# qwerty35/swarm_simulator

Hardware: AMD Instinct MI355X
Metric: agent-trajectories/sec (RBP plan: SFC+RSFC+QP) (higher is better)
Workload: dtype f64

## Files before the change

### swarm_simulator_amd/csrc/kernels/knot_lds.inc

```
#pragma once
#include "knot_panel_layout.h"

#define KL_LD 38
#define KL_LDU 50
#define KL_I 40
#ifndef KL_XCH
#define KL_XCH 6
#endif
typedef __attribute__((address_space(3))) double kl_lds;
typedef __attribute__((address_space(3))) int kl_ldsi;
typedef double kl_d2 __attribute__((ext_vector_type(2)));
typedef __attribute__((address_space(3))) kl_d2 kl_lds2;
typedef double kl_d4 __attribute__((ext_vector_type(4)));

__host__ __device__ constexpr int kl_area_doubles(int nk) {
    return ((nk + 1) * KL_LDU + (nk + 1) * KL_LD + KL_I + 1) & ~1;
}

template <int NK>
struct KlArea {
    static constexpr int NT = (NK + 15) / 16;
    static constexpr int C = 0, CSZ = (NK + 1) * KL_LDU;
    static constexpr int MX = CSZ, MXSZ = (NK + 1) * KL_LD;
    static constexpr int I = MX + MXSZ;
// ... 562 lines not shown
        return dinv;
    } else {
#pragma unroll
        for (int k = 0; k < NK; ++k) m[k] = (k == r) ? 1.0 : 0.0;
        if (FOLLOW)
            kl_follow_LinvT<NK>(m, C, I, P, pbase);
        else
            kl_row_times_LinvT<NK>(m, C, I);
        if (FOLLOW) kl_await_opaque(P, pbase + NK + 1);
        const double dinv = I[act ? r : 0];
        kl_store_rows<NK>(m, MX, r, act);
        if (FOLLOW) kl_publish(Mdone, done_value);
        return dinv;
    }
}
```

### swarm_simulator_amd/csrc/kernels/qp.hip

```cpp
#include <algorithm>
#include <type_traits>
#include <vector>

#include "rbp_dev.h"

#pragma clang fp contract(fast)

#include "knot_lds.inc"
#include "common/ipm_rows.h"

#ifndef QP_THREADS
#define QP_THREADS 512
#endif
#define QP_MAX_ITERS 80
#ifndef QP_WARM_TAU
#define QP_WARM_TAU 1e-3
#endif
#ifndef QP_MU0
#define QP_MU0 3e-1
#endif
#ifndef QP_ROW_UNROLL
#define QP_ROW_UNROLL 2
#endif
#ifndef QP_ROW_PF
// ... 25 lines not shown
#endif
#ifndef QP_WAVES_PER_EU
#define QP_WAVES_PER_EU 2
#endif
#ifndef QP_CHAIN_PRIO
#define QP_CHAIN_PRIO 3
#endif
#ifndef QP_STAGE_BUFS
#define QP_STAGE_BUFS (QP_THREADS >= 512 ? 3 : 2)
#endif
#ifndef QP_STAGE_REGS
#define QP_STAGE_REGS (QP_THREADS >= 512 ? 0 : 2)
#endif
#ifndef QP_MID_FOLLOW
#define QP_MID_FOLLOW (QP_THREADS >= 512)
#endif
#ifndef QP_EARLY_TRIES
#define QP_EARLY_TRIES 2
#endif
#ifndef QP_EARLY_TOL
#define QP_EARLY_TOL 1e-6
#endif
#include "lh_layout.h"
#define PL_NC 256
#define PL_PMAX 160
#define PL_PBIG 192
__host__ __device__ inline int polish_pmax(int nk) { return nk <= 36 ? 112 : PL_PMAX; }
__host__ __device__ inline size_t polish_s_doubles(int nj) { return std::max((size_t)PL_NC * PL_NC, ipm::k0g_doubles(nj)); }
__host__ __device__ inline size_t polish_ws_doubles(int nj, int nk) {
    return 18 * (size_t)nj + 2 + ipm::k0g_doubles(nj) + PL_NC * 14 + polish_s_doubles(nj) + 8 + lhp_size(PL_PBIG) + 4 * 6 * PL_PBIG + 3 * (size_t)nj * nk;
// ... 1392 lines not shown
    c.w = carve(ws_base + (size_t)mission * ws_stride, c.d, nbmax);
    double* ctrl = S.ctrl + (size_t)mission * N * 3 * 6 * MS;
    c.ctrl = ctrl;
    c.normals = S.rsfc_normal + (size_t)mission * S.npair * MS * 3;
    c.radius = S.radius + (size_t)mission * N;
    const QpDims& d = c.d;
    const QpWs& w = c.w;
    const double* T = S.T + (size_t)mission * (MS + 1);
    double* scal = S.scalars + (size_t)mission * SC_N;

    extern __shared__ __attribute__((aligned(16))) double lds_raw[];
    double* red = lds_raw;
    int* flag = (int*)(lds_raw + 16);
    double* lds = lds_raw + 32;
#ifdef QP_PROFILE
    const BlkArgs ba{d.nk, d.nj, d.ldb, c.lds_avail, w.Td, w.To, w.Lf, w.Ek, scal};
#else
    const BlkArgs ba{d.nk, d.nj, d.ldb, c.lds_avail, w.Td, w.To, w.Lf, w.Ek, nullptr};
#endif

    PROF_DECL;
    int frozen_free_rows = 0, nfar = 0;
    if (!qp_setup_batch(S, c, ctrl, T, mission, first, nb, flag, lds, frozen_free_rows, far_R, nfar)) return 0;
    PROF(8);
    PassIO io;
    __shared__ RowCtx c_lds;
#if QP_ROW_BLK > 0
    __shared__ SweepMeta meta_lds;
    const bool meta_ok = nb * d.M <= QP_META_G && d.ntile + 1 <= 16 && d.N <= 256 && (size_t)nb * d.M * d.N < 65536;
    __syncthreads();
    if (meta_ok) {
        for (int rk = tid; rk < nb * d.M; rk += QP_THREADS) {
            const int g = w.fperm[rk];
// ... 13 lines not shown
    const double pin_viol = block_reduce(io.vmax, 1, red);
    if (pin_viol > 1e-6) {
        if (tid == 0) {
            atomicCAS(&S.status[mission], 0, (int)RBP_ERR_QP_FAILED);
#ifndef QP_PROFILE
            scal[SC_PROF0 + 1] = 1000.0 * batch + 1, scal[SC_PROF0 + 2] = pin_viol;
#endif
        }
        return 0;
    }
    const double nrows_free = (double)((size_t)(d.oq - 6) * (6 * d.nb + d.npb)) + (double)frozen_free_rows;
    bool ok = false;
    int it_count = 0, polished = 0, early_tries = 0, fail_reason = 3;
    double gap_next = 0, pres_next = 0, kkt_ipm = 0;
    double flops = 0, rows_swept = 0, row_bytes = 0, sweep_bytes = 0;
    const double blk_doubles = d.nk <= 36 ? 5.0 * (d.nk * (d.nk + 1) / 2) + 5.0 * d.nk : 8.0 * d.ldb * d.ldb;
    const double bytes_sweeps = 88.0 * frozen_free_rows + 64.0 * (double)(d.oq - 6) * (6.0 * d.nb + 2.0 * d.npb) + 288.0 * (double)d.nb * (d.oq - 6);
    const double bytes_iter = bytes_sweeps + 8.0 * (double)d.nj * blk_doubles;
    const PolishWs pw = polish_carve(w.polish, d.nj);
    row_pass<PASS_INIT>(c, io);
    __threadfence_block();
    __syncthreads();
#ifdef QP_TRACE
    double* trc = S.coef + (size_t)mission * N * 3 * 6 * MS;
#endif
    for (int iter = 0; iter < QP_MAX_ITERS; ++iter) {
        it_count = iter;
        PROF(0);
        if (iter == 0) {
            io.sum0 = 0, io.vmax = 0;
            SWEEP(PASS_BUILD);
// ... 31 lines not shown
            const int acc = polish_entry(c, pw, lds, red, flag, polish_first ? 1 : 0);
            __syncthreads();
            PROF(0);
#ifdef QP_POLSTATS
            if (tid == 0 && !polish_first) scal[25] += (early_tries == 1), scal[26] += (early_tries == 1 && acc == 0), scal[27] += (early_tries == 2), scal[29] += (early_tries == 2 && acc == 0);
#endif
            if (acc == 0) {
                ok = true, polished = 1;
                break;
            }
        }
        if (d.nk > 36)
            assemble_blocks(c, lds);
        else if (ASM_HELPERS == 0 && !QP_FOLLOW_ASM)
            assemble_blocks_lds(asm_args(c), d.nj, lds);
        PROF(3);
        __threadfence_block();
        __syncthreads();
        TRC(5, trc_sum(w.Td, (size_t)d.nj * d.ldb * d.ldb, red));
        if (!factor_entry(ba, asm_args(c), lds, flag)) {
            fail_reason = 2;
            break;
        }
        flops += d.nk <= 36 ? (double)d.nj * ((7.0 / 6.0) * d.nk * (double)d.nk * d.nk + 6.0 * d.nk * (double)d.nk)
                            : (double)d.nj * (7.0 / 3.0) * d.nk * (double)d.nk * d.nk;
        PROF(4);
        TRC(6, trc_sum(d.nk <= 36 ? w.Lf : w.Td, d.nk <= 36 ? (size_t)d.nj * 2 * d.nk * d.nk : (size_t)d.nj * d.ldb * d.ldb, red));
#ifndef QP_TRACE
        if (d.nk <= 36) {
            PROF(5);
            solve_entry(ba, w.rhs, lds, SolveOut{w.dxa, w.Lk, d.oq, 1, w.cpacc, w.rbase, 0.0});
            PROF(6);
        } else
#endif
        {
            rhs_from_acc(c, false, 0.0);
            __threadfence_block();
            __syncthreads();
            PROF(5);
            TRC(7, trc_sum(w.rhs, (size_t)d.nj * d.nk, red));
            solve_entry(ba, w.rhs, lds);
            PROF(6);
            TRC(8, trc_sum(w.rhs, (size_t)d.nj * d.nk, red));
            apply_F(d, w, w.rhs, w.dxa);
            __threadfence_block();
            __syncthreads();
// ... 303 lines not shown
```

### swarm_simulator_amd/csrc/kernels/qp_base.inc

```

#ifdef QP_PROFILE
#define PROF_DECL long long prof_t0 = wall_clock64(), prof_acc[12] = {0, 0, 0, 0, 0, 0, 0, 0, 0, 0, 0, 0}
#define PROF(i)                                \
    do {                                       \
        __syncthreads();                       \
        long long t_ = wall_clock64();         \
        prof_acc[i] += t_ - prof_t0;           \
        prof_t0 = t_;                          \
    } while (0)
#define PROF_FLUSH(scal)                                                         \
    do {                                                                         \
        if (threadIdx.x == 0)                                                    \
            for (int i_ = 0; i_ < 12; ++i_) scal[SC_PROF0 + i_] += (double)prof_acc[i_]; \
    } while (0)
#else
#define PROF_DECL
#define PROF(i)
#define PROF_FLUSH(scal)
#endif

struct QpDims {
    int N, M, oq;
    int nb, NF, npb;
    int nk, nj, ld;
// ... 117 lines not shown
    v = wave_red(v, op);
    const int wave = threadIdx.x >> 6, lane = threadIdx.x & 63;
    if (lane == 0) red[wave] = v;
    __syncthreads();
    double r = red[0];
    for (int i = 1; i < QP_THREADS / 64; ++i) r = red_op(r, red[i], op);
    __syncthreads();
    return r;
}

struct BlkArgs {
    int nk, nj, ldb, lds_avail;
    double *Td, *To, *Lf;
    double* Ek;
    double* prof;
};
__device__ __forceinline__ int uni(int v) { return __builtin_amdgcn_readfirstlane(v); }
template <class T>
__device__ __forceinline__ T* uni(T* p) {
    const unsigned long long v = (unsigned long long)p;
    const unsigned lo = __builtin_amdgcn_readfirstlane((unsigned)v), hi = __builtin_amdgcn_readfirstlane((unsigned)(v >> 32));
    return (T*)(((unsigned long long)hi << 32) | lo);
}
__device__ __forceinline__ void blk_unpack(const BlkArgs& b, QpDims& d, QpWs& w) {
    d = QpDims{};
    w = QpWs{};
    d.nk = uni(b.nk), d.nj = uni(b.nj), d.ldb = uni(b.ldb), d.ld = d.nk + 1;
    w.Td = uni(b.Td), w.To = uni(b.To), w.Lf = uni(b.Lf), w.Ek = uni(b.Ek), w.prof = uni(b.prof);
}
template <class T>
__device__ __forceinline__ T uni_words(const T& v) {
    static_assert(sizeof(T) % 4 == 0, "whole words");
    union U {
        T t;
        unsigned wd[sizeof(T) / 4];
        __device__ U() {}
    } in, out;
    in.t = v;
#pragma unroll
    for (unsigned i = 0; i < sizeof(T) / 4; ++i) out.wd[i] = __builtin_amdgcn_readfirstlane(in.wd[i]);
    return out.t;
}

// ... 48 lines not shown
```

### swarm_simulator_amd/csrc/kernels/qp_wave_factor.inc

```

__device__ __forceinline__ int twist_mid(int nj) { return nj / 2; }

#define ASM_WAVE0 4
#define ASM_HELPERS (QP_THREADS / 64 > ASM_WAVE0 ? QP_THREADS / 64 - ASM_WAVE0 : 0)
#ifndef QP_FOLLOW_ASM
#define QP_FOLLOW_ASM (ASM_HELPERS == 0)
#endif
#define ASMF_READY(cnt, h) ((kl_ldsi*)((cnt) + 76 + (h)))
__device__ __forceinline__ void wait_blocks(int* cnt, int i) {
    while (__hip_atomic_load(cnt + i, __ATOMIC_RELAXED, __HIP_MEMORY_SCOPE_WORKGROUP) < ASM_HELPERS) __builtin_amdgcn_s_sleep(2);
    __builtin_amdgcn_fence(__ATOMIC_ACQUIRE, "workgroup");
}

typedef double d4 __attribute__((ext_vector_type(4)));

template <int NK>
__device__ __forceinline__ bool chol_rows(double (&a)[NK], double& dinv) {
    bool ok = true;
    const int r = threadIdx.x & 63;
    dinv = 1.0;
#pragma unroll
    for (int c = 0; c < NK; ++c) {
        const double dcc = rl(a[c], c);
        if (!(dcc > 0)) ok = false;
// ... 96 lines not shown

#if defined(QP_PROFILE) && !defined(QP_LHSTATS) && !defined(QP_SOLVE_TIMERS)
#define CHAIN_TW(cnt, slot) ((__attribute__((address_space(3))) unsigned long long*)((cnt) + 96) + ((slot) - 25))
#define CHAIN_T0 long long ct_ = wall_clock64()
#define CHAIN_T(slot)                                                                                                                              \
    do {                                                                                                                                           \
        const long long t_ = wall_clock64();                                                                                                       \
        __hip_atomic_fetch_add(CHAIN_TW(cnt, slot), (dir > 0 && r == 0) ? (unsigned long long)(t_ - ct_) : 0ull, __ATOMIC_RELAXED, __HIP_MEMORY_SCOPE_WORKGROUP); \
        ct_ = t_;                                                                                                                                  \
    } while (0)
#define CHAIN_FLUSH()                                                                                   \
    do {                                                                                                \
        kl_sync();                                                                                      \
        if (w.prof && dir > 0 && r == 0)                                                                \
            for (int k_ = 25; k_ < 28; ++k_) w.prof[k_] += (double)(long long)*CHAIN_TW(cnt, k_);       \
    } while (0)
#else
#define CHAIN_T0
#define CHAIN_T(slot)
#define CHAIN_FLUSH()
#endif
#define CHAIN_SYNC(cnt, h) ((kl_ldsi*)((cnt) + 64 + 2 * (h)))
#define ASM_CONSUMED(cnt, h) ((kl_ldsi*)((cnt) + 72 + (h)))

template <int NK>
__device__ __forceinline__ bool wave_factor_chain(const QpDims& d, const QpWs& w, int j0, int count, int dir, double* ldsW, int* cnt, int h) {
    using A = KlArea<NK>;
    kl_lds* base = (kl_lds*)ldsW;
    kl_lds *MX = base + A::MX, *I = base + A::I, *U = base + A::C;
    kl_ldsi *P = CHAIN_SYNC(cnt, h), *Mdone = P + 1;
    const int r = threadIdx.x & 63;
    const bool act = r < NK;
    const int rr = act ? r : 0;
    bool ok = true;
    int seen = 0, seen_img = 0;
    if constexpr (kl_fused_path(NK)) {
        double cf[KlPanels<NK>::NT][3];
        for (int i = 0, j = j0; i < count; ++i, j += dir) {
            CHAIN_T0;
            kl_d4 s[KlPanels<NK>::TILES];
            kl_tiles_zero<NK>(s);
            if (i > 0) {
                kl_await(Mdone, i, seen);
                CHAIN_T(27);
                kl_fused_update<NK>(s, MX, I, r, cf);
            }
            CHAIN_T(25);
            if (QP_FOLLOW_ASM)
                kl_await(ASMF_READY(cnt, h), i + 1, seen_img);
            else
                wait_blocks(cnt, i);
            CHAIN_T(26);
            fused_coupling_coef<NK>(w, j, dir, r, cf);
            const kl_lds* Timg = ASM_HELPERS > 0 ? (const kl_lds*)(ldsW - (size_t)h * A::SIZE + 2 * A::SIZE + 128 + (size_t)(h + 2 * (i & 1)) * ASML_DOUBLES(NK, (NK / 9)))
                                 : QP_FOLLOW_ASM ? (const kl_lds*)(ldsW - (size_t)h * A::SIZE + 2 * A::SIZE + 128 + (size_t)h * ASML_DOUBLES(NK, (NK / 9)))
                                                 : nullptr;
            if (!knot_ldl_add<NK>(w, j, s, base, r, P, i * (NK + 1), Timg, ASM_CONSUMED(cnt, h), i + 1)) ok = false;
            CHAIN_T(27);
        }
        CHAIN_FLUSH();
        return ok;
    }
    for (int i = 0, j = j0; i < count; ++i, j += dir) {
        CHAIN_T0;
        if (i > 0) kl_syrk<NK>(MX, I, U, r, false);
        CHAIN_T(25);
        if (QP_FOLLOW_ASM)
            kl_await(ASMF_READY(cnt, h), i + 1, seen_img);
        else
            wait_blocks(cnt, i);
        CHAIN_T(26);
        double e0, e1, e2, x[NK];
        coupling_coef(w, j, dir, rr, e0, e1, e2);
// ... 44 lines not shown
        kl_await(ASMF_READY(cnt, 0), mid + 1, seen_img);
    } else {
        wait_blocks(cnt, cnt_idx);
    }
    kl_ldsi* scratch = CHAIN_SYNC(cnt, 2);
    const kl_lds* Timg = ASM_HELPERS > 0 ? (const kl_lds*)(ldsL + 2 * A::SIZE + 128 + (size_t)(2 * (cnt_idx & 1)) * ASML_DOUBLES(NK, (NK / 9)))
                         : QP_FOLLOW_ASM ? (const kl_lds*)(ldsL + 2 * A::SIZE + 128) : nullptr;
    bool ok;
    if constexpr (kl_fused_path(NK))
        ok = knot_ldl_add<NK>(w, mid, s, bl, r, scratch, 0, Timg);
    else
        ok = knot_ldl<NK>(w, mid, nsy > 0, bl, r, act, rr, scratch, 0, Timg);
    if (!QP_MID_FOLLOW) {
        int seen = 0;
        knot_inverse<NK, false>(w, mid, bl, r, act, scratch, 0, seen, scratch, 0);
    }
    return ok;
}

template <int NK, int ROLE>
__device__ __forceinline__ bool twisted_factor(const QpDims& d, const QpWs& w, int* flag, double* lds, const AsmArgs* asmb) {
    const int wave = (ROLE == 0 || ROLE == 2) ? (threadIdx.x >> 6) & 1 : 4, mid = twist_mid(d.nj);
    const int nl = mid, nr = d.nj - 1 - mid, SF = nl > nr ? nl : nr;
    constexpr int AREA = KlArea<NK>::SIZE;
    int* cnt = (int*)(lds + 2 * AREA);
    static_assert((QP_MAX_M - 1) / 2 + 1 <= 64, "cnt[0..SF] must end below CHAIN_SYNC (cnt + 64): sessions with M > QP_MAX_M are refused");
    if (threadIdx.x == 0) *flag = 0;
    __syncthreads();
    bool ok = true;
    for (int i = threadIdx.x; i < 2 * AREA + 64; i += QP_THREADS) lds[i] = 0.0;
// ... 85 lines not shown
```

### swarm_simulator_amd/csrc/kernels/qp_wave_solve.inc

```

#define KS_VPAD 16
#define KS_VLEN (KS_VPAD + KL_I + KS_VPAD)
template <int NK>
struct KsPieces {
    static constexpr int CH = (NK * 15 + 35) / 36;
    static constexpr int N0 = NK, N1 = NK - CH > 0 ? NK - CH : 0, N2 = NK - 2 * CH > 0 ? NK - 2 * CH : 0;
    static_assert(NK - 3 * CH <= 0 && N0 + N1 + N2 <= 64, "three chunks, one wavefront");
    static_assert(3 * CH - NK <= KS_VPAD && 3 * CH - 1 - (NK - 1) <= KS_VPAD, "vector padding");
    __device__ static __forceinline__ void of_lane(int lane, int& idx, int& t) {
        t = lane < N0 ? 0 : (lane < N0 + N1 ? 1 : 2);
        idx = lane < N0 ? lane : (lane < N0 + N1 ? lane - N0 : (lane < N0 + N1 + N2 ? lane - N0 - N1 : 0));
    }
};
template <int NK>
__device__ __forceinline__ double kl_matvec_cols(const kl_lds* Mst, const kl_lds* b, kl_lds* psum, int lane) {
    using P = KsPieces<NK>;
    int idx, t;
    P::of_lane(lane, idx, t);
    const int k0 = P::CH * t, c = k0 + idx;
    const kl_lds* mp = Mst + k0 * KL_LD + c;
    const kl_lds* bp = b + k0;
    double mv[P::CH], bv[P::CH];
#pragma unroll
    for (int j = 0; j < P::CH; ++j) mv[j] = mp[j * KL_LD], bv[j] = bp[j];
    double s0 = 0, s1 = 0, s2 = 0;
#pragma unroll
    for (int j = 0; j < P::CH; ++j) {
        if (j % 3 == 0) s0 += mv[j] * bv[j];
        if (j % 3 == 1) s1 += mv[j] * bv[j];
        if (j % 3 == 2) s2 += mv[j] * bv[j];
    }
    psum[lane] = (s0 + s1) + s2;
    kl_sync();
    const int cc = lane < NK ? lane : 0;
    double r = psum[cc];
    if (P::N1 > 0) r += cc >= P::CH ? psum[P::N0 + cc - P::CH] : 0.0;
    if (P::N2 > 0) r += cc >= 2 * P::CH ? psum[P::N0 + P::N1 + cc - 2 * P::CH] : 0.0;
    return r;
}
template <int NK>
__device__ __forceinline__ double kl_matvec_rows(const kl_lds* Mst, const kl_lds* b, kl_lds* psum, int lane) {
    using P = KsPieces<NK>;
    int idx, t;
    P::of_lane(lane, idx, t);
    const int k0 = NK - P::CH * (t + 1);
    const kl_lds* mp = Mst + idx * KL_LD + k0;
    const kl_lds* bp = b + k0;
    double mv[P::CH], bv[P::CH];
#pragma unroll
    for (int j = 0; j < P::CH; ++j) mv[j] = mp[j], bv[j] = bp[j];
    double s0 = 0, s1 = 0, s2 = 0;
#pragma unroll
    for (int j = 0; j < P::CH; ++j) {
        if (j % 3 == 0) s0 += mv[j] * bv[j];
        if (j % 3 == 1) s1 += mv[j] * bv[j];
        if (j % 3 == 2) s2 += mv[j] * bv[j];
    }
    psum[lane] = (s0 + s1) + s2;
    kl_sync();
    const int rr = lane < NK ? lane : 0;
    double r = psum[rr];
    if (P::N1 > 0) r += rr < P::N1 ? psum[P::N0 + rr] : 0.0;
    if (P::N2 > 0) r += rr < P::N2 ? psum[P::N0 + P::N1 + rr] : 0.0;
    return r;
}

template <int NK>
struct KsLayout {
    static constexpr int SM = NK * KL_LD, SCH = SM + KL_I, STG = 2 * SCH;
    static constexpr int LEAD = 16;
    static constexpr int VECS = 6 * KS_VLEN + 2 * 64;
};

struct SolveOut {
    double* dx_out;
    const double* Lk;
    int oq;
    int rhs_mode = 0;
    const double* cpacc = nullptr;
    const double* rbase = nullptr;
    double sigma_mu = 0;
};
template <int NK, int ROLE>
__device__ __forceinline__ void solve_staged(const QpDims& d, const QpWs& w, double* rhs, double* lds, SolveOut so = SolveOut{nullptr, nullptr, 0}) {
    using KS = KsLayout<NK>;
    constexpr int STG = KS::STG, SCH = KS::SCH, SM = KS::SM;
    const int tid = threadIdx.x, nj = d.nj, mid = twist_mid(nj);
    const int nl = mid, nr = nj - 1 - mid, SF = nl > nr ? nl : nr;
    const int nsteps = 2 * SF + 1;
    lds += KS::LEAD;
    kl_lds* vec = (kl_lds*)(lds + QP_STAGE_BUFS * STG);
    kl_lds* small = vec + ((nj * NK + 1) & ~1);
    if (so.rhs_mode) {
        constexpr int nu = NK / 3;
        const int oq = so.oq;
        const size_t ncp = (size_t)(NK / 9) * oq;
        const bool corrector = so.rhs_mode == 2;
        for (int it = tid; it < nj * nu; it += QP_THREADS) {
            const int j = it / nu + 1, u = it % nu, a = u / 3, k = u % 3;
            double g[6];
#pragma unroll
            for (int q = 0; q < 6; ++q) {
                const int j6 = 6 * (j - 1) + 3 + q;
                const __attribute__((address_space(1))) double* ac = QGC(so.cpacc) + (size_t)a * oq + j6;
                g[q] = corrector ? ac[k * ncp] - so.sigma_mu * ac[(3 + k) * ncp] : ac[(6 + k) * ncp];
            }
            const __attribute__((address_space(1))) double* L = QGC(so.Lk) + 9 * j;
            const size_t o0 = (size_t)(j - 1) * NK + u * 3;
// ... 25 lines not shown
                const int side = e >= NE, idx = side ? e - NE : e;
                if (idx < NTRI) {
                    int rw = (int)(((2 * NK + 1) - sqrtf((float)((2 * NK + 1) * (2 * NK + 1) - 8 * idx))) * 0.5f);
                    if (rw * NK - rw * (rw - 1) / 2 > idx) rw--;
                    if ((rw + 1) * NK - (rw + 1) * rw / 2 <= idx) rw++;
                    const int k = rw + idx - (rw * NK - rw * (rw - 1) / 2);
                    soff[u] = rw * NK + k, doff[u] = side * SCH + rw * KL_LD + k;
                } else {
                    soff[u] = NK * NK + (idx - NTRI), doff[u] = side * SCH + SM + (idx - NTRI);
                }
            }
        }
    }
    for (int i = tid; i < KS::LEAD + QP_STAGE_BUFS * STG; i += QP_THREADS) (lds - KS::LEAD)[i] = 0.0;
    __syncthreads();
    auto stage = [&](int s, double* buf) {
        const int jl = left_j(s), jr = right_j(s);
        const double* srcl = w.Lf + (size_t)(jl >= 0 ? jl : 0) * KF_STRIDE(NK);
        const double* srcr = w.Lf + (size_t)(jr >= 0 ? jr : 0) * KF_STRIDE(NK);
        double tmp[MAXE];
#pragma unroll
        for (int u = 0; u < MAXE; ++u) {
            const bool right = doff[u] >= SCH;
            const bool on = doff[u] >= 0 && (right ? jr >= 0 : jl >= 0);
            tmp[u] = on ? (right ? srcr : srcl)[soff[u]] : 0.0;
        }
#pragma unroll
        for (int u = 0; u < MAXE; ++u) {
            const bool right = doff[u] >= SCH;
            if (doff[u] >= 0 && (right ? jr >= 0 : jl >= 0)) buf[doff[u]] = tmp[u];
// ... 7 lines not shown
        gdbl* srcr = (gdbl*)(w.Lf + (size_t)(jr >= 0 ? jr : 0) * KF_STRIDE(NK));
#pragma unroll
        for (int u = 0; u < MAXE; ++u) tmp[u] = (doff[u] >= SCH ? srcr : srcl)[soff[u]];
    };
    auto stage_store = [&](int s, const double (&tmp)[MAXE], double* buf) {
        if (s >= nsteps) return;
        const int jl = left_j(s), jr = right_j(s);
        kl_lds* bl = (kl_lds*)buf;
#pragma unroll
        for (int u = 0; u < MAXE; ++u) {
            const bool right = doff[u] >= SCH;
            if (doff[u] >= 0 && (right ? jr >= 0 : jl >= 0)) bl[doff[u]] = tmp[u];
        }
    };
    if (ROLE == 1)
        for (int s0 = 0; s0 < QP_STAGE_BUFS - 1 && s0 < nsteps; ++s0) stage(s0, lds + s0 * STG);
    __syncthreads();
    const int wave = ROLE == 0 ? (tid >> 6) & 1 : 2, r = tid & 63;
    const bool act = r < NK;
    const int rr = act ? r : 0, g3 = 3 * (rr / 3), r3 = rr % 3;
    const int rs = act ? r : NK + 12;
    if (wave < 2) __builtin_amdgcn_s_setprio(QP_CHAIN_PRIO);
    auto step_coef = [&](int s, double& q0, double& q1, double& q2) {
        q0 = q1 = q2 = 0.0;
        if (ROLE != 0 || s >= nsteps || s == SF) return;
        const int jb = wave == 0 ? left_j(s) : right_j(s);
        if (jb < 0) return;
        const int dir = wave == 0 ? +1 : -1;
        if (s < SF) {
            const bool has_prev = wave == 0 ? jb > 0 : jb + 1 < nj;
            if (has_prev) coupling_coef(w, jb - dir, dir, rr, q0, q1, q2);
        } else {
            const __attribute__((address_space(1))) double* E = QGC(w.Ek) + 9 * (dir > 0 ? jb + 1 : jb);
            q0 = dir > 0 ? E[3 * r3] : E[r3], q1 = dir > 0 ? E[3 * r3 + 1] : E[3 + r3], q2 = dir > 0 ? E[3 * r3 + 2] : E[6 + r3];
        }
    };
    double cf0, cf1, cf2;
    step_coef(0, cf0, cf1, cf2);
#ifdef QP_SOLVE_TIMERS
    long long st_ = wall_clock64();
#define SOLVE_T(slot)                                                              \
    do {                                                                           \
        const long long t_ = wall_clock64();                                       \
        const int who_ = ROLE == 0 ? (tid == 0 ? 0 : (tid == 64 ? 8 : -1)) : (tid == 128 ? 4 : -1);  \
        if (w.prof && who_ >= 0) w.prof[slot + who_] += (double)(t_ - st_);        \
        st_ = t_;                                                                  \
    } while (0)
#else
#define SOLVE_T(slot)
#endif
    if (ROLE == 1 && QP_STAGE_REGS > 0) {
        constexpr int R = QP_STAGE_REGS > 0 ? QP_STAGE_REGS : 1;
        double tq[R][MAXE];
#pragma unroll
        for (int k = 0; k < R; ++k) stage_load(QP_STAGE_BUFS - 1 + k, tq[k]);
        int dsto[MAXE];
#pragma unroll
        for (int u = 0; u < MAXE; ++u) dsto[u] = doff[u] >= 0 ? doff[u] : KL_LD - 1;
        typedef __attribute__((address_space(1))) const double gdbl;
        double nq[R][MAXE];
        int s = 0;
        for (; s + 2 * R + QP_STAGE_BUFS - 1 <= nsteps; s += R) {
#pragma unroll
            for (int k = 0; k < R; ++k) {
                const int sl = s + R + k + QP_STAGE_BUFS - 1;
                const int jl = left_j(sl), jr = right_j(sl);
                gdbl* srcl = (gdbl*)(w.Lf + (size_t)(jl >= 0 ? jl : 0) * KF_STRIDE(NK));
                gdbl* srcr = (gdbl*)(w.Lf + (size_t)(jr >= 0 ? jr : 0) * KF_STRIDE(NK));
#pragma unroll
                for (int u = 0; u < MAXE; ++u) nq[k][u] = (doff[u] >= SCH ? srcr : srcl)[soff[u]];
            }
#pragma unroll
            for (int k = 0; k < R; ++k) {
                const int sp = s + k + QP_STAGE_BUFS - 1;
                kl_lds* bl = (kl_lds*)(lds + (sp % QP_STAGE_BUFS) * STG);
#pragma unroll
// ... 5 lines not shown
#pragma unroll
                for (int u = 0; u < MAXE; ++u) tq[k][u] = nq[k][u];
        }
        for (; s < nsteps; s += R) {
#pragma unroll
            for (int k = 0; k < R; ++k) {
                if (s + k < nsteps) {
                    const int sp = s + k + QP_STAGE_BUFS - 1;
                    stage_store(sp, tq[k], lds + (sp % QP_STAGE_BUFS) * STG);
                    stage_load(sp + R, tq[k]);
                    __syncthreads();
                }
            }
        }
    } else
    for (int s = 0; s < nsteps; ++s) {
        SOLVE_T(26);
        const double e0 = cf0, e1 = cf1, e2 = cf2;
        step_coef(s + 1, cf0, cf1, cf2);
        double* buf = lds + (s % QP_STAGE_BUFS) * STG;
        if (ROLE == 1) {
            const int sp = s + QP_STAGE_BUFS - 1;
            if (sp < nsteps) stage(sp, lds + (sp % QP_STAGE_BUFS) * STG);
        } else if (s == SF) {
            if (wave == 0) {
                const kl_lds* Mst = (const kl_lds*)buf;
                kl_lds *A0 = (kl_lds*)small + KS_VPAD, *Z0 = A0 + KS_VLEN, *V0 = A0 + 2 * KS_VLEN, *V1 = A0 + 5 * KS_VLEN;
                kl_lds* ps = (kl_lds*)small + 6 * KS_VLEN;
                double v = vec[mid * NK + rr];
                if (mid > 0) {
                    double e0, e1, e2;
                    coupling_coef(w, mid - 1, +1, rr, e0, e1, e2);
                    v -= e0 * V0[g3] + e1 * V0[g3 + 1] + e2 * V0[g3 + 2];
                }
                if (mid + 1 < nj) {
                    double e0, e1, e2;
                    coupling_coef(w, mid + 1, -1, rr, e0, e1, e2);
                    v -= e0 * V1[g3] + e1 * V1[g3 + 1] + e2 * V1[g3 + 2];
                }
                A0[rs] = v;
                kl_sync();
                const double z = Mst[SM + rr] * kl_matvec_cols<NK>(Mst, A0, ps, r);
                Z0[rs] = z;
                kl_sync();
                const double x = kl_matvec_rows<NK>(Mst, Z0, ps, r);
                kl_sync();
                V0[rs] = x, V1[rs] = x;
                if (act) vec[mid * NK + r] = x;
            }
        } else {
            const bool fwd = s < SF;
            const int jb = wave == 0 ? left_j(s) : right_j(s);
            if (jb >= 0) {
                const kl_lds* Mst = (const kl_lds*)(buf + (wave == 0 ? 0 : SCH));
                kl_lds *A = (kl_lds*)small + KS_VPAD + (wave == 0 ? 0 : 3 * KS_VLEN), *Z = A + KS_VLEN, *V = A + 2 * KS_VLEN;
                kl_lds* ps = (kl_lds*)small + 6 * KS_VLEN + (wave == 0 ? 0 : 64);
                const double dinv = Mst[SM + rr];
                if (fwd) {
                    double v = vec[jb * NK + rr];
                    const bool has_prev = wave == 0 ? jb > 0 : jb + 1 < nj;
                    if (has_prev) v -= e0 * V[g3] + e1 * V[g3 + 1] + e2 * V[g3 + 2];
                    kl_sync();
                    A[rs] = v;
                    kl_sync();
                    const double z = dinv * kl_matvec_cols<NK>(Mst, A, ps, r);
                    Z[rs] = z;
                    if (act) vec[jb * NK + r] = z;
                    kl_sync();
                    const double vj = kl_matvec_rows<NK>(Mst, Z, ps, r);
                    kl_sync();
                    V[rs] = vj;
                } else {
                    const double wv = e0 * V[g3] + e1 * V[g3 + 1] + e2 * V[g3 + 2];
                    kl_sync();
                    A[rs] = wv;
                    kl_sync();
                    const double u = vec[jb * NK + rr] - dinv * kl_matvec_cols<NK>(Mst, A, ps, r);
                    Z[rs] = u;
                    kl_sync();
                    const double x = kl_matvec_rows<NK>(Mst, Z, ps, r);
                    kl_sync();
                    V[rs] = x;
                    if (act) vec[jb * NK + r] = x;
                }
            }
        }
        SOLVE_T(25);
        __syncthreads();
    }
    if (wave < 2) __builtin_amdgcn_s_setprio(0);
    if (so.dx_out) {
        constexpr int nu = NK / 3;
        const int oq = so.oq;
        for (int it = tid; it < nj * nu; it += QP_THREADS) {
            const int j = it / nu + 1, u = it % nu;
            const kl_lds* uu = vec + (size_t)(j - 1) * NK + u * 3;
            const __attribute__((address_space(1))) double* L = QGC(so.Lk) + 9 * j;
// ... 18 lines not shown
```

Baseline: 188,100.

## Fuse forward substitution and middle solve into the NK=36 factor chain

For nk==36 on the fused panel path, the forward-substitution step for each knot block is performed inside the wave factor chain right after that block is factored, and the twisted middle solve runs at the end of factorization. The separate solve then runs only the backward half (rhs_mode 3), skipping the forward stages and their staging of factor panels from global memory. It refactors the shared matvec and step helpers into a common header and adds per-step LDS slots in the C region, which adds work and synchronization to the factor critical path in exchange for removing a pass over the factors.

```diff
diff --git a/swarm_simulator_amd/csrc/kernels/knot_lds.inc b/swarm_simulator_amd/csrc/kernels/knot_lds.inc
--- a/swarm_simulator_amd/csrc/kernels/knot_lds.inc
+++ b/swarm_simulator_amd/csrc/kernels/knot_lds.inc
@@ -600,3 +600,23 @@
         return dinv;
     }
 }
+
+#include "knot_subst.h"
+template <int NK>
+__device__ __forceinline__ void kl_forward_step(kl_lds* base, __attribute__((address_space(1))) double* z_out, double rhs_r, double e0, double e1, double e2, int r) {
+    using A = KlArea<NK>;
+    using F = KfSlots<NK>;
+    static_assert(F::CSZ == A::CSZ, "knot_subst.h out of step with KlArea");
+    kl_lds *C = base + A::C, *MX = base + A::MX, *I = base + A::I;
+    const int rr = r < NK ? r : 0, g3 = 3 * (rr / 3);
+    ks_step_forward<NK, true>((const kl_lds*)MX, I[rr], rhs_r, true, e0, e1, e2, C + F::A, C + F::Z, C + F::V, C + F::PS, r, g3, rr, [] { kl_sync(); },
+                              [&](double z) { *z_out = z; });
+}
+template <int NK>
+__device__ __forceinline__ double kl_middle_step(kl_lds* base, double v, int r) {
+    using A = KlArea<NK>;
+    using F = KfSlots<NK>;
+    kl_lds* C = base + A::C;
+    const int rr = r < NK ? r : 0;
+    return ks_step_middle<NK, true>((const kl_lds*)(base + A::MX), (const kl_lds*)(base + A::I + rr), v, C + F::A, C + F::Z, C + F::PS, r, rr, [] { kl_sync(); });
+}
diff --git a/swarm_simulator_amd/csrc/kernels/knot_subst.h b/swarm_simulator_amd/csrc/kernels/knot_subst.h
--- /dev/null
+++ b/swarm_simulator_amd/csrc/kernels/knot_subst.h
@@ -0,0 +1,133 @@
+#pragma once
+#include "knot_panel_layout.h"
+#ifndef KS_FN
+#define KS_FN __host__ __device__ __forceinline__
+#endif
+#ifndef KL_LD
+#define KL_LD 38
+#endif
+#ifndef KL_I
+#define KL_I 40
+#endif
+#ifndef KL_LDU
+#define KL_LDU 50
+#endif
+#define KS_VPAD 16
+#define KS_VLEN (KS_VPAD + KL_I + KS_VPAD)
+template <int NK>
+struct KsPieces {
+    static constexpr int CH = (NK * 15 + 35) / 36;
+    static constexpr int N0 = NK, N1 = NK - CH > 0 ? NK - CH : 0, N2 = NK - 2 * CH > 0 ? NK - 2 * CH : 0;
+    static_assert(NK - 3 * CH <= 0 && N0 + N1 + N2 <= 64, "three chunks, one wavefront");
+    static_assert(3 * CH - NK <= KS_VPAD && 3 * CH - 1 - (NK - 1) <= KS_VPAD, "vector padding");
+    static KS_FN void of_lane(int lane, int& idx, int& t) {
+        t = lane < N0 ? 0 : (lane < N0 + N1 ? 1 : 2);
+        idx = lane < N0 ? lane : (lane < N0 + N1 ? lane - N0 : (lane < N0 + N1 + N2 ? lane - N0 - N1 : 0));
+    }
+};
+template <int NK, bool GUARD = false, class MP, class VP, class PP, class SY>
+KS_FN double ks_matvec_cols(MP Mst, VP b, PP psum, int lane, SY&& sync) {
+    using P = KsPieces<NK>;
+    int idx, t;
+    P::of_lane(lane, idx, t);
+    const int k0 = P::CH * t, c = k0 + idx;
+    const auto mp = Mst + k0 * KL_LD + c;
+    const auto bp = b + k0;
+    double mv[P::CH], bv[P::CH];
+#pragma unroll
+    for (int j = 0; j < P::CH; ++j) {
+        mv[j] = mp[j * KL_LD], bv[j] = bp[j];
+        if (GUARD && 2 * P::CH + j > NK) mv[j] = k0 + j > NK ? 0.0 : mv[j];
+    }
+    double s0 = 0, s1 = 0, s2 = 0;
+#pragma unroll
+    for (int j = 0; j < P::CH; ++j) {
+        if (j % 3 == 0) s0 += mv[j] * bv[j];
+        if (j % 3 == 1) s1 += mv[j] * bv[j];
+        if (j % 3 == 2) s2 += mv[j] * bv[j];
+    }
+    psum[lane] = (s0 + s1) + s2;
+    sync();
+    const int cc = lane < NK ? lane : 0;
+    double r = psum[cc];
+    if (P::N1 > 0) r += cc >= P::CH ? psum[P::N0 + cc - P::CH] : 0.0;
+    if (P::N2 > 0) r += cc >= 2 * P::CH ? psum[P::N0 + P::N1 + cc - 2 * P::CH] : 0.0;
+    return r;
+}
+template <int NK, class MP, class VP, class PP, class SY>
+KS_FN double ks_matvec_rows(MP Mst, VP b, PP psum, int lane, SY&& sync) {
+    using P = KsPieces<NK>;
+    int idx, t;
+    P::of_lane(lane, idx, t);
+    const int k0 = NK - P::CH * (t + 1);
+    const auto mp = Mst + idx * KL_LD + k0;
+    const auto bp = b + k0;
+    double mv[P::CH], bv[P::CH];
+#pragma unroll
+    for (int j = 0; j < P::CH; ++j) mv[j] = mp[j], bv[j] = bp[j];
+    double s0 = 0, s1 = 0, s2 = 0;
+#pragma unroll
+    for (int j = 0; j < P::CH; ++j) {
+        if (j % 3 == 0) s0 += mv[j] * bv[j];
+        if (j % 3 == 1) s1 += mv[j] * bv[j];
+        if (j % 3 == 2) s2 += mv[j] * bv[j];
+    }
+    psum[lane] = (s0 + s1) + s2;
+    sync();
+    const int rr = lane < NK ? lane : 0;
+    double r = psum[rr];
+    if (P::N1 > 0) r += rr < P::N1 ? psum[P::N0 + rr] : 0.0;
+    if (P::N2 > 0) r += rr < P::N2 ? psum[P::N0 + P::N1 + rr] : 0.0;
+    return r;
+}
+
+template <int NK, bool GUARD = false, class MP, class VP, class PP, class SY, class ZF>
+KS_FN void ks_step_forward(MP Mst, double dinv, double rhs_r, bool has_prev, double e0, double e1, double e2, VP A, VP Z, VP V, PP ps, int lane, int g3, int rs,
+                           SY&& sync, ZF&& put_z) {
+    double v = rhs_r;
+    if (has_prev) v -= e0 * V[g3] + e1 * V[g3 + 1] + e2 * V[g3 + 2];
+    sync();
+    A[rs] = v;
+    sync();
+    const double z = dinv * ks_matvec_cols<NK, GUARD>(Mst, A, ps, lane, sync);
+    Z[rs] = z;
+    put_z(z);
+    sync();
+    const double vj = ks_matvec_rows<NK>(Mst, Z, ps, lane, sync);
+    sync();
+    V[rs] = vj;
+}
+KS_FN double ks_couple(double e0, double e1, double e2, double v0, double v1, double v2) { return e0 * v0 + e1 * v1 + e2 * v2; }
+template <int NK, bool GUARD = false, class MP, class DP, class VP, class PP, class SY>
+KS_FN double ks_step_middle(MP Mst, DP dinv_p, double v, VP A0, VP Z0, PP ps, int lane, int rs, SY&& sync) {
+    A0[rs] = v;
+    sync();
+    const double z = dinv_p[0] * ks_matvec_cols<NK, GUARD>(Mst, A0, ps, lane, sync);
+    Z0[rs] = z;
+    sync();
+    const double x = ks_matvec_rows<NK>(Mst, Z0, ps, lane, sync);
+    sync();
+    return x;
+}
+template <int NK, bool GUARD = false, class MP, class ZP, class VP, class PP, class SY>
+KS_FN double ks_step_backward(MP Mst, double dinv, ZP z_p, double e0, double e1, double e2, VP A, VP Z, VP V, PP ps, int lane, int g3, int rs, SY&& sync) {
+    const double wv = e0 * V[g3] + e1 * V[g3 + 1] + e2 * V[g3 + 2];
+    sync();
+    A[rs] = wv;
+    sync();
+    const double u = z_p[0] - dinv * ks_matvec_cols<NK, GUARD>(Mst, A, ps, lane, sync);
+    Z[rs] = u;
+    sync();
+    const double x = ks_matvec_rows<NK>(Mst, Z, ps, lane, sync);
+    sync();
+    V[rs] = x;
+    return x;
+}
+
+template <int NK>
+struct KfSlots {
+    static constexpr int CSZ = (NK + 1) * KL_LDU;
+    static constexpr int PAD = kp_img_total(NK), Z = PAD + 10, V = Z + NK, END = V + NK, A = PAD - NK, PS = A - 64;
+    static_assert(KsPieces<NK>::CH * 3 - NK <= 10, "the run of zeros between A and Z");
+    static_assert(END + 9 <= CSZ && PS >= kp_img_off(NK, kp_np(NK) - 1), "forward-step vectors: tail of the C region, end of the last panel image");
+};
diff --git a/swarm_simulator_amd/csrc/kernels/qp.hip b/swarm_simulator_amd/csrc/kernels/qp.hip
--- a/swarm_simulator_amd/csrc/kernels/qp.hip
+++ b/swarm_simulator_amd/csrc/kernels/qp.hip
@@ -63,6 +63,18 @@
 #endif
 #ifndef QP_MID_FOLLOW
 #define QP_MID_FOLLOW (QP_THREADS >= 512)
+#endif
+#ifndef QP_FWD_IN_FACTOR
+#ifdef QP_TRACE
+#define QP_FWD_IN_FACTOR 0
+#else
+#define QP_FWD_IN_FACTOR 1
+#endif
+#endif
+#if QP_FWD_IN_FACTOR && KL_FUSED_UPDATE && KL_PANEL && KL_PANEL_MIN_NK <= 36
+#define QP_FWD36 1
+#else
+#define QP_FWD36 0
 #endif
 #ifndef QP_EARLY_TRIES
 #define QP_EARLY_TRIES 2
@@ -1485,9 +1497,17 @@
     int* flag = (int*)(lds_raw + 16);
     double* lds = lds_raw + 32;
 #ifdef QP_PROFILE
+#if QP_FWD36
+    const BlkArgs ba{d.nk, d.nj, d.ldb, c.lds_avail, w.Td, w.To, w.Lf, w.Ek, scal, w.rhs};
+#else
     const BlkArgs ba{d.nk, d.nj, d.ldb, c.lds_avail, w.Td, w.To, w.Lf, w.Ek, scal};
+#endif
+#else
+#if QP_FWD36
+    const BlkArgs ba{d.nk, d.nj, d.ldb, c.lds_avail, w.Td, w.To, w.Lf, w.Ek, nullptr, w.rhs};
 #else
     const BlkArgs ba{d.nk, d.nj, d.ldb, c.lds_avail, w.Td, w.To, w.Lf, w.Ek, nullptr};
+#endif
 #endif
 
     PROF_DECL;
@@ -1531,7 +1551,11 @@
     int it_count = 0, polished = 0, early_tries = 0, fail_reason = 3;
     double gap_next = 0, pres_next = 0, kkt_ipm = 0;
     double flops = 0, rows_swept = 0, row_bytes = 0, sweep_bytes = 0;
+#if QP_FWD36
+    const double blk_doubles = d.nk == 36 ? 4.5 * (d.nk * (d.nk + 1) / 2) + 4.5 * d.nk : (d.nk < 36 ? 5.0 * (d.nk * (d.nk + 1) / 2) + 5.0 * d.nk : 8.0 * d.ldb * d.ldb);
+#else
     const double blk_doubles = d.nk <= 36 ? 5.0 * (d.nk * (d.nk + 1) / 2) + 5.0 * d.nk : 8.0 * d.ldb * d.ldb;
+#endif
     const double bytes_sweeps = 88.0 * frozen_free_rows + 64.0 * (double)(d.oq - 6) * (6.0 * d.nb + 2.0 * d.npb) + 288.0 * (double)d.nb * (d.oq - 6);
     const double bytes_iter = bytes_sweeps + 8.0 * (double)d.nj * blk_doubles;
     const PolishWs pw = polish_carve(w.polish, d.nj);
@@ -1593,6 +1617,9 @@
             assemble_blocks(c, lds);
         else if (ASM_HELPERS == 0 && !QP_FOLLOW_ASM)
             assemble_blocks_lds(asm_args(c), d.nj, lds);
+#if QP_FWD36
+        if (d.nk == 36) rhs_from_acc(c, false, 0.0);
+#endif
         PROF(3);
         __threadfence_block();
         __syncthreads();
@@ -1608,7 +1635,11 @@
 #ifndef QP_TRACE
         if (d.nk <= 36) {
             PROF(5);
+            #if QP_FWD36
+            solve_entry(ba, w.rhs, lds, SolveOut{w.dxa, w.Lk, d.oq, d.nk == 36 ? 3 : 1, w.cpacc, w.rbase, 0.0});
+#else
             solve_entry(ba, w.rhs, lds, SolveOut{w.dxa, w.Lk, d.oq, 1, w.cpacc, w.rbase, 0.0});
+#endif
             PROF(6);
         } else
 #endif
diff --git a/swarm_simulator_amd/csrc/kernels/qp_base.inc b/swarm_simulator_amd/csrc/kernels/qp_base.inc
--- a/swarm_simulator_amd/csrc/kernels/qp_base.inc
+++ b/swarm_simulator_amd/csrc/kernels/qp_base.inc
@@ -155,6 +155,9 @@
     double *Td, *To, *Lf;
     double* Ek;
     double* prof;
+#if QP_FWD36
+    double* rhs;
+#endif
 };
 __device__ __forceinline__ int uni(int v) { return __builtin_amdgcn_readfirstlane(v); }
 template <class T>
@@ -168,6 +171,9 @@
     w = QpWs{};
     d.nk = uni(b.nk), d.nj = uni(b.nj), d.ldb = uni(b.ldb), d.ld = d.nk + 1;
     w.Td = uni(b.Td), w.To = uni(b.To), w.Lf = uni(b.Lf), w.Ek = uni(b.Ek), w.prof = uni(b.prof);
+#if QP_FWD36
+    w.rhs = uni(b.rhs);
+#endif
 }
 template <class T>
 __device__ __forceinline__ T uni_words(const T& v) {
diff --git a/swarm_simulator_amd/csrc/kernels/qp_wave_factor.inc b/swarm_simulator_amd/csrc/kernels/qp_wave_factor.inc
--- a/swarm_simulator_amd/csrc/kernels/qp_wave_factor.inc
+++ b/swarm_simulator_amd/csrc/kernels/qp_wave_factor.inc
@@ -134,6 +134,7 @@
         kl_sync();                                                                                      \
         if (w.prof && dir > 0 && r == 0)                                                                \
             for (int k_ = 25; k_ < 28; ++k_) w.prof[k_] += (double)(long long)*CHAIN_TW(cnt, k_);       \
+        if (QP_FWD_IN_FACTOR && w.prof && dir > 0 && r == 0) w.prof[29] += (double)(long long)*CHAIN_TW(cnt, 29); \
     } while (0)
 #else
 #define CHAIN_T0
@@ -142,6 +143,19 @@
 #endif
 #define CHAIN_SYNC(cnt, h) ((kl_ldsi*)((cnt) + 64 + 2 * (h)))
 #define ASM_CONSUMED(cnt, h) ((kl_ldsi*)((cnt) + 72 + (h)))
+
+static_assert((QP_FWD36 != 0) == (QP_FWD_IN_FACTOR && kl_fused_path(36)), "QP_FWD36 (qp.hip) out of step with kl_fused_path");
+template <int NK>
+__device__ __forceinline__ void wave_forward_step(const QpWs& w, kl_lds* base, int jp, double rhs_r, double e0, double e1, double e2, int r) {
+    kl_forward_step<NK>(base, QG(w.rhs) + (size_t)jp * NK + (r < NK ? r : 0), rhs_r, e0, e1, e2, r);
+}
+template <int NK>
+__device__ __forceinline__ void wave_forward_fetch(const QpWs& w, int j, int dir, bool first, int r, double& rhs_r, double& e0, double& e1, double& e2) {
+    const int rr = r < NK ? r : 0;
+    rhs_r = QGC(w.rhs)[(size_t)j * NK + rr];
+    coupling_coef(w, first ? j : j - dir, dir, rr, e0, e1, e2);
+    e0 = first ? 0.0 : e0, e1 = first ? 0.0 : e1, e2 = first ? 0.0 : e2;
+}
 
 template <int NK>
 __device__ __forceinline__ bool wave_factor_chain(const QpDims& d, const QpWs& w, int j0, int count, int dir, double* ldsW, int* cnt, int h) {
@@ -156,6 +170,7 @@
     int seen = 0, seen_img = 0;
     if constexpr (kl_fused_path(NK)) {
         double cf[KlPanels<NK>::NT][3];
+        [[maybe_unused]] double f_rhs = 0, f_e0 = 0, f_e1 = 0, f_e2 = 0;
         for (int i = 0, j = j0; i < count; ++i, j += dir) {
             CHAIN_T0;
             kl_d4 s[KlPanels<NK>::TILES];
@@ -166,6 +181,10 @@
                 kl_fused_update<NK>(s, MX, I, r, cf);
             }
             CHAIN_T(25);
+            if (QP_FWD_IN_FACTOR) {
+                if (i > 0) wave_forward_step<NK>(w, base, j - dir, f_rhs, f_e0, f_e1, f_e2, r);
+                CHAIN_T(29);
+            }
             if (QP_FOLLOW_ASM)
                 kl_await(ASMF_READY(cnt, h), i + 1, seen_img);
             else
@@ -176,7 +195,15 @@
                                  : QP_FOLLOW_ASM ? (const kl_lds*)(ldsW - (size_t)h * A::SIZE + 2 * A::SIZE + 128 + (size_t)h * ASML_DOUBLES(NK, (NK / 9)))
                                                  : nullptr;
             if (!knot_ldl_add<NK>(w, j, s, base, r, P, i * (NK + 1), Timg, ASM_CONSUMED(cnt, h), i + 1)) ok = false;
+            if (QP_FWD_IN_FACTOR) wave_forward_fetch<NK>(w, j, dir, i == 0, r, f_rhs, f_e0, f_e1, f_e2);
             CHAIN_T(27);
+        }
+        if (QP_FWD_IN_FACTOR) {
+            CHAIN_T0;
+            kl_await(Mdone, count, seen);
+            CHAIN_T(27);
+            wave_forward_step<NK>(w, base, j0 + (count - 1) * dir, f_rhs, f_e0, f_e1, f_e2, r);
+            CHAIN_T(29);
         }
         CHAIN_FLUSH();
         return ok;
@@ -251,6 +278,28 @@
     if (!QP_MID_FOLLOW) {
         int seen = 0;
         knot_inverse<NK, false>(w, mid, bl, r, act, scratch, 0, seen, scratch, 0);
+    }
+    if constexpr (QP_FWD_IN_FACTOR && kl_fused_path(NK)) {
+        using F = KfSlots<NK>;
+        if (QP_MID_FOLLOW) {
+            int seen = 0;
+            kl_await(scratch + 1, 1, seen);
+        }
+        const kl_lds *V0 = bl + A::C + F::V, *V1 = br + A::C + F::V;
+        const int g3 = 3 * (rr / 3);
+        double v = QGC(w.rhs)[(size_t)mid * NK + rr];
+        if (mid > 0) {
+            double e0, e1, e2;
+            coupling_coef(w, mid - 1, +1, rr, e0, e1, e2);
+            v -= e0 * V0[g3] + e1 * V0[g3 + 1] + e2 * V0[g3 + 2];
+        }
+        if (mid + 1 < d.nj) {
+            double e0, e1, e2;
+            coupling_coef(w, mid + 1, -1, rr, e0, e1, e2);
+            v -= e0 * V1[g3] + e1 * V1[g3 + 1] + e2 * V1[g3 + 2];
+        }
+        const double x = kl_middle_step<NK>(bl, v, r);
+        QG(w.rhs)[(size_t)mid * NK + rr] = x;
     }
     return ok;
 }
diff --git a/swarm_simulator_amd/csrc/kernels/qp_wave_solve.inc b/swarm_simulator_amd/csrc/kernels/qp_wave_solve.inc
--- a/swarm_simulator_amd/csrc/kernels/qp_wave_solve.inc
+++ b/swarm_simulator_amd/csrc/kernels/qp_wave_solve.inc
@@ -1,69 +1,5 @@
 
-#define KS_VPAD 16
-#define KS_VLEN (KS_VPAD + KL_I + KS_VPAD)
-template <int NK>
-struct KsPieces {
-    static constexpr int CH = (NK * 15 + 35) / 36;
-    static constexpr int N0 = NK, N1 = NK - CH > 0 ? NK - CH : 0, N2 = NK - 2 * CH > 0 ? NK - 2 * CH : 0;
-    static_assert(NK - 3 * CH <= 0 && N0 + N1 + N2 <= 64, "three chunks, one wavefront");
-    static_assert(3 * CH - NK <= KS_VPAD && 3 * CH - 1 - (NK - 1) <= KS_VPAD, "vector padding");
-    __device__ static __forceinline__ void of_lane(int lane, int& idx, int& t) {
-        t = lane < N0 ? 0 : (lane < N0 + N1 ? 1 : 2);
-        idx = lane < N0 ? lane : (lane < N0 + N1 ? lane - N0 : (lane < N0 + N1 + N2 ? lane - N0 - N1 : 0));
-    }
-};
-template <int NK>
-__device__ __forceinline__ double kl_matvec_cols(const kl_lds* Mst, const kl_lds* b, kl_lds* psum, int lane) {
-    using P = KsPieces<NK>;
-    int idx, t;
-    P::of_lane(lane, idx, t);
-    const int k0 = P::CH * t, c = k0 + idx;
-    const kl_lds* mp = Mst + k0 * KL_LD + c;
-    const kl_lds* bp = b + k0;
-    double mv[P::CH], bv[P::CH];
-#pragma unroll
-    for (int j = 0; j < P::CH; ++j) mv[j] = mp[j * KL_LD], bv[j] = bp[j];
-    double s0 = 0, s1 = 0, s2 = 0;
-#pragma unroll
-    for (int j = 0; j < P::CH; ++j) {
-        if (j % 3 == 0) s0 += mv[j] * bv[j];
-        if (j % 3 == 1) s1 += mv[j] * bv[j];
-        if (j % 3 == 2) s2 += mv[j] * bv[j];
-    }
-    psum[lane] = (s0 + s1) + s2;
-    kl_sync();
-    const int cc = lane < NK ? lane : 0;
-    double r = psum[cc];
-    if (P::N1 > 0) r += cc >= P::CH ? psum[P::N0 + cc - P::CH] : 0.0;
-    if (P::N2 > 0) r += cc >= 2 * P::CH ? psum[P::N0 + P::N1 + cc - 2 * P::CH] : 0.0;
-    return r;
-}
-template <int NK>
-__device__ __forceinline__ double kl_matvec_rows(const kl_lds* Mst, const kl_lds* b, kl_lds* psum, int lane) {
-    using P = KsPieces<NK>;
-    int idx, t;
-    P::of_lane(lane, idx, t);
-    const int k0 = NK - P::CH * (t + 1);
-    const kl_lds* mp = Mst + idx * KL_LD + k0;
-    const kl_lds* bp = b + k0;
-    double mv[P::CH], bv[P::CH];
-#pragma unroll
-    for (int j = 0; j < P::CH; ++j) mv[j] = mp[j], bv[j] = bp[j];
-    double s0 = 0, s1 = 0, s2 = 0;
-#pragma unroll
-    for (int j = 0; j < P::CH; ++j) {
-        if (j % 3 == 0) s0 += mv[j] * bv[j];
-        if (j % 3 == 1) s1 += mv[j] * bv[j];
-        if (j % 3 == 2) s2 += mv[j] * bv[j];
-    }
-    psum[lane] = (s0 + s1) + s2;
-    kl_sync();
-    const int rr = lane < NK ? lane : 0;
-    double r = psum[rr];
-    if (P::N1 > 0) r += rr < P::N1 ? psum[P::N0 + rr] : 0.0;
-    if (P::N2 > 0) r += rr < P::N2 ? psum[P::N0 + P::N1 + rr] : 0.0;
-    return r;
-}
+#include "knot_subst.h"
 
 template <int NK>
 struct KsLayout {
@@ -88,10 +24,13 @@
     const int tid = threadIdx.x, nj = d.nj, mid = twist_mid(nj);
     const int nl = mid, nr = nj - 1 - mid, SF = nl > nr ? nl : nr;
     const int nsteps = 2 * SF + 1;
+    constexpr bool FWD = QP_FWD_IN_FACTOR && kl_fused_path(NK);
+    const bool bwd_only = FWD && so.rhs_mode == 3;
+    const int s_first = bwd_only ? SF + 1 : 0;
     lds += KS::LEAD;
     kl_lds* vec = (kl_lds*)(lds + QP_STAGE_BUFS * STG);
     kl_lds* small = vec + ((nj * NK + 1) & ~1);
-    if (so.rhs_mode) {
+    if (FWD ? so.rhs_mode == 1 || so.rhs_mode == 2 : so.rhs_mode != 0) {
         constexpr int nu = NK / 3;
         const int oq = so.oq;
         const size_t ncp = (size_t)(NK / 9) * oq;
@@ -147,6 +86,7 @@
     }
     for (int i = tid; i < KS::LEAD + QP_STAGE_BUFS * STG; i += QP_THREADS) (lds - KS::LEAD)[i] = 0.0;
     __syncthreads();
+    if (bwd_only && tid < NK) small[KS_VPAD + 2 * KS_VLEN + tid] = small[KS_VPAD + 5 * KS_VLEN + tid] = vec[mid * NK + tid];
     auto stage = [&](int s, double* buf) {
         const int jl = left_j(s), jr = right_j(s);
         const double* srcl = w.Lf + (size_t)(jl >= 0 ? jl : 0) * KF_STRIDE(NK);
@@ -184,7 +124,7 @@
         }
     };
     if (ROLE == 1)
-        for (int s0 = 0; s0 < QP_STAGE_BUFS - 1 && s0 < nsteps; ++s0) stage(s0, lds + s0 * STG);
+        for (int s0 = s_first; s0 < s_first + QP_STAGE_BUFS - 1 && s0 < nsteps; ++s0) stage(s0, lds + (bwd_only ? s0 % QP_STAGE_BUFS : s0) * STG);
     __syncthreads();
     const int wave = ROLE == 0 ? (tid >> 6) & 1 : 2, r = tid & 63;
     const bool act = r < NK;
@@ -206,7 +146,7 @@
         }
     };
     double cf0, cf1, cf2;
-    step_coef(0, cf0, cf1, cf2);
+    step_coef(s_first, cf0, cf1, cf2);
 #ifdef QP_SOLVE_TIMERS
     long long st_ = wall_clock64();
 #define SOLVE_T(slot)                                                              \
@@ -223,13 +163,13 @@
         constexpr int R = QP_STAGE_REGS > 0 ? QP_STAGE_REGS : 1;
         double tq[R][MAXE];
 #pragma unroll
-        for (int k = 0; k < R; ++k) stage_load(QP_STAGE_BUFS - 1 + k, tq[k]);
+        for (int k = 0; k < R; ++k) stage_load(s_first + QP_STAGE_BUFS - 1 + k, tq[k]);
         int dsto[MAXE];
 #pragma unroll
         for (int u = 0; u < MAXE; ++u) dsto[u] = doff[u] >= 0 ? doff[u] : KL_LD - 1;
         typedef __attribute__((address_space(1))) const double gdbl;
         double nq[R][MAXE];
-        int s = 0;
+        int s = s_first;
         for (; s + 2 * R + QP_STAGE_BUFS - 1 <= nsteps; s += R) {
 #pragma unroll
             for (int k = 0; k < R; ++k) {
@@ -265,7 +205,7 @@
             }
         }
     } else
-    for (int s = 0; s < nsteps; ++s) {
+    for (int s = s_first; s < nsteps; ++s) {
         SOLVE_T(26);
         const double e0 = cf0, e1 = cf1, e2 = cf2;
         step_coef(s + 1, cf0, cf1, cf2);
@@ -289,13 +229,7 @@
                     coupling_coef(w, mid + 1, -1, rr, e0, e1, e2);
                     v -= e0 * V1[g3] + e1 * V1[g3 + 1] + e2 * V1[g3 + 2];
                 }
-                A0[rs] = v;
-                kl_sync();
-                const double z = Mst[SM + rr] * kl_matvec_cols<NK>(Mst, A0, ps, r);
-                Z0[rs] = z;
-                kl_sync();
-                const double x = kl_matvec_rows<NK>(Mst, Z0, ps, r);
-                kl_sync();
+                const double x = ks_step_middle<NK>(Mst, Mst + SM + rr, v, A0, Z0, ps, r, rs, [] { kl_sync(); });
                 V0[rs] = x, V1[rs] = x;
                 if (act) vec[mid * NK + r] = x;
             }
@@ -308,30 +242,12 @@
                 kl_lds* ps = (kl_lds*)small + 6 * KS_VLEN + (wave == 0 ? 0 : 64);
                 const double dinv = Mst[SM + rr];
                 if (fwd) {
-                    double v = vec[jb * NK + rr];
                     const bool has_prev = wave == 0 ? jb > 0 : jb + 1 < nj;
-                    if (has_prev) v -= e0 * V[g3] + e1 * V[g3 + 1] + e2 * V[g3 + 2];
-                    kl_sync();
-                    A[rs] = v;
-                    kl_sync();
-                    const double z = dinv * kl_matvec_cols<NK>(Mst, A, ps, r);
-                    Z[rs] = z;
-                    if (act) vec[jb * NK + r] = z;
-                    kl_sync();
-                    const double vj = kl_matvec_rows<NK>(Mst, Z, ps, r);
-                    kl_sync();
-                    V[rs] = vj;
+                    ks_step_forward<NK>(Mst, dinv, vec[jb * NK + rr], has_prev, e0, e1, e2, A, Z, V, ps, r, g3, rs, [] { kl_sync(); }, [&](double z) {
+                        if (act) vec[jb * NK + r] = z;
+                    });
                 } else {
-                    const double wv = e0 * V[g3] + e1 * V[g3 + 1] + e2 * V[g3 + 2];
-                    kl_sync();
-                    A[rs] = wv;
-                    kl_sync();
-                    const double u = vec[jb * NK + rr] - dinv * kl_matvec_cols<NK>(Mst, A, ps, r);
-                    Z[rs] = u;
-                    kl_sync();
-                    const double x = kl_matvec_rows<NK>(Mst, Z, ps, r);
-                    kl_sync();
-                    V[rs] = x;
+                    const double x = ks_step_backward<NK>(Mst, dinv, vec + jb * NK + rr, e0, e1, e2, A, Z, V, ps, r, g3, rs, [] { kl_sync(); });
                     if (act) vec[jb * NK + r] = x;
                 }
             }
```

After: 190,200 (median of 6 runs). 1.1% higher.
